# JBLanier/stratego_env

Measured on AMD Instinct MI355X. Metric: env steps/sec, higher is better.
Workload: dtype u8

## Files before the change

stratego_env_amd/csrc/sgx_choose.h:

```cpp
#pragma once

namespace {

constexpr int CHOOSE_BITS = 23;
constexpr uint32_t CHOOSE_ONE = 1u << CHOOSE_BITS;

template <class G, int VEC>
struct ChooseGeo {
    static constexpr int NA = G::NA;
    static constexpr int NCH = (NA + VEC - 1) / VEC;
    static constexpr int ROWS = (NCH + G::LPG - 1) / G::LPG;
    static constexpr bool CACHE = ROWS * VEC <= 72;
    static constexpr int WAVES = 4, GAMES = WAVES * G::GPW;
};

__device__ __forceinline__ uint32_t choose_weight(float l, float mx, float scale) {
    const uint32_t w = (uint32_t)exp2f(fmaf(l - mx, scale, (float)CHOOSE_BITS));
    return l == mx ? CHOOSE_ONE : w;
}

template <class G>
__device__ __forceinline__ uint32_t gsum(uint32_t c) {
    if constexpr (G::LPG == 64) {
        int x = (int)c;
        x += dpp_or_zero<0x111>(x);
        x += dpp_or_zero<0x112>(x);
        x += dpp_or_zero<0x114>(x);
        x += dpp_or_zero<0x118>(x);
        return (uint32_t)__builtin_amdgcn_readlane(x, 15) + (uint32_t)__builtin_amdgcn_readlane(x, 31) +
               (uint32_t)__builtin_amdgcn_readlane(x, 47) + (uint32_t)__builtin_amdgcn_readlane(x, 63);
    } else {
        return (uint32_t)glane<G>(gscan_incl<G>((int)c), G::LPG - 1);
    }
}

template <class G>
__device__ __forceinline__ float gmax(float x) {
#pragma unroll
    for (int o = G::LPG / 2; o > 0; o >>= 1) x = fmaxf(x, __shfl_xor(x, o, G::LPG));
    return x;
}

template <int R_, int C_, int VEC, bool BITS>
__global__ __launch_bounds__(256) void choose_kernel(const KParams P, const float *__restrict__ logits, const void *__restrict__ mask, const float scale,
                                                     int32_t *__restrict__ actions) {
    using G = Geo<R_, C_>;
    using CG = ChooseGeo<G, VEC>;
    constexpr int NA = CG::NA, ROWS = CG::ROWS, LPG = G::LPG;
    __shared__ uint32_t rowtot[CG::GAMES][CG::CACHE ? 1 : ROWS];
    const int lane = threadIdx.x & (LPG - 1), slot = threadIdx.x / LPG;
    const int64_t env = blockIdx.x * (int64_t)CG::GAMES + slot;
    if (env >= P.n_envs) return;
    const float *lg = logits + env * (int64_t)NA;
    const uint8_t *mb = BITS ? nullptr : reinterpret_cast<const uint8_t *>(mask) + env * (int64_t)NA;
    const uint32_t *mw = BITS ? reinterpret_cast<const uint32_t *>(mask) + env * (int64_t)G::MB_WORDS : nullptr;
    const int4 sc = rec_scal<G>(P.boards, P.rec_bytes, env)[0];

    auto load_row = [&](int j, float (&v)[VEC], bool stream) {
        const int ch = j * LPG + lane, i = ch * VEC;
#pragma unroll
        for (int e = 0; e < VEC; ++e) v[e] = -INFINITY;
        if (i >= NA) return;
        uint32_t vm;
        if constexpr (VEC == 4) {
            const f32x4 q = stream ? __builtin_nontemporal_load(reinterpret_cast<const f32x4 *>(lg) + ch) : reinterpret_cast<const f32x4 *>(lg)[ch];
            v[0] = q.x; v[1] = q.y; v[2] = q.z; v[3] = q.w;
            if constexpr (BITS) vm = (mw[i >> 5] >> (i & 31)) & 15u;
            else {
                const uint32_t m4 = reinterpret_cast<const uint32_t *>(mb)[ch];
                vm = ((m4 & 0xFFu) ? 1u : 0u) | ((m4 & 0xFF00u) ? 2u : 0u) | ((m4 & 0xFF0000u) ? 4u : 0u) | ((m4 & 0xFF000000u) ? 8u : 0u);
            }
        } else {
            v[0] = stream ? __builtin_nontemporal_load(lg + i) : lg[i];
            if constexpr (BITS) vm = (mw[i >> 5] >> (i & 31)) & 1u;
            else vm = mb[i] ? 1u : 0u;
        }
#pragma unroll
        for (int e = 0; e < VEC; ++e)
            if (!((vm >> e) & 1u) || !(v[e] == v[e])) v[e] = -INFINITY;
    };
    auto chunk_sum = [&](const float (&v)[VEC], float mx) {
        uint32_t c = 0;
#pragma unroll
        for (int e = 0; e < VEC; ++e) c += choose_weight(v[e], mx, scale);
        return c;
    };

    float cv[CG::CACHE ? ROWS : 1][VEC];
    float mx = -INFINITY;
    if constexpr (CG::CACHE) {
#pragma unroll
        for (int j = 0; j < ROWS; ++j) load_row(j, cv[j], true);
#pragma unroll
        for (int j = 0; j < ROWS; ++j)
#pragma unroll
            for (int e = 0; e < VEC; ++e) mx = fmaxf(mx, cv[j][e]);
    } else {
        for (int j = 0; j < ROWS; ++j) {
            float v[VEC];
            load_row(j, v, false);
#pragma unroll
            for (int e = 0; e < VEC; ++e) mx = fmaxf(mx, v[e]);
        }
    }
    mx = gmax<G>(mx);
    if (mx == -INFINITY) {
        if (lane == 0) actions[env] = -1;
        return;
    }

    const uint64_t r = sgx_rng(P.seed, (uint64_t)(P.env_id_offset + env), (uint64_t)sc.w, STREAM_ACTION, (uint32_t)sc.x);
    unsigned long long total = 0, target = 0, before = 0;
    int jr = 0;
    if constexpr (CG::CACHE) {
        uint32_t t[ROWS];
#pragma unroll
        for (int j = 0; j < ROWS; ++j) { t[j] = gsum<G>(chunk_sum(cv[j], mx)); total += t[j]; }
        target = __umul64hi((r >> 32) << 32, total);
        bool found = false;
#pragma unroll
        for (int j = 0; j < ROWS; ++j) {
            if (!found && before + t[j] > target) { jr = j; found = true; }
            if (!found) before += t[j];
        }
    } else {
        for (int j = 0; j < ROWS; ++j) {
            float v[VEC];
            load_row(j, v, false);
            const uint32_t t = gsum<G>(chunk_sum(v, mx));
            if (lane == 0) rowtot[slot][j] = t;
            total += t;
        }
        wave_sync<G>();
        target = __umul64hi((r >> 32) << 32, total);
        for (int j = 0; j < ROWS; ++j) {
            const uint32_t t = rowtot[slot][j];
            if (before + t > target) { jr = j; break; }
            before += t;
        }
    }
    float v[VEC];
    load_row(jr, v, false);
    uint32_t w[VEC], c = 0;
#pragma unroll
    for (int e = 0; e < VEC; ++e) { w[e] = choose_weight(v[e], mx, scale); c += w[e]; }
    const unsigned long long incl = before + (unsigned long long)(uint32_t)gscan_incl<G>((int)c);
    const unsigned long long hit = gballot<G>(incl > target);
    const int l = __ffsll((long long)hit) - 1;
    if (lane == l) {
        unsigned long long cum = incl - c;
        int pick = VEC - 1;
        bool found = false;
#pragma unroll
        for (int e = 0; e < VEC; ++e) {
            cum += w[e];
            if (!found && cum > target) { pick = e; found = true; }
        }
        actions[env] = (jr * LPG + lane) * VEC + pick;
    }
}

}
```

Baseline: 260.8 million.

## Load masks first and skip logit loads and reductions for fully masked rows

The action sampler now reads the legal-action mask for a group of rows first, then fetches logits only for lanes with legal actions. Rows where no lane in the wave has a legal action skip the max, the weight computation and the group-sum reduction. Uncached rows are processed in fixed-size groups so loads can batch. This targets sparse Stratego masks where most logits are illegal, at the cost of extra ballots, bit packing and more complex control flow.

```diff
diff --git a/stratego_env_amd/csrc/sgx_choose.h b/stratego_env_amd/csrc/sgx_choose.h
--- a/stratego_env_amd/csrc/sgx_choose.h
+++ b/stratego_env_amd/csrc/sgx_choose.h
@@ -12,6 +12,8 @@
     static constexpr int ROWS = (NCH + G::LPG - 1) / G::LPG;
     static constexpr bool CACHE = ROWS * VEC <= 72;
     static constexpr int WAVES = 4, GAMES = WAVES * G::GPW;
+    static constexpr int GR = CACHE ? ROWS : VEC == 4 ? 8 : 16;
+    static constexpr int NG = (ROWS + GR - 1) / GR, VW = (GR * VEC + 31) / 32, RW = (GR + 31) / 32;
 };
 
 __device__ __forceinline__ uint32_t choose_weight(float l, float mx, float scale) {
@@ -56,29 +58,58 @@
     const uint32_t *mw = BITS ? reinterpret_cast<const uint32_t *>(mask) + env * (int64_t)G::MB_WORDS : nullptr;
     const int4 sc = rec_scal<G>(P.boards, P.rec_bytes, env)[0];
 
-    auto load_row = [&](int j, float (&v)[VEC], bool stream) {
+    auto load_valid = [&](int j) -> uint32_t {
         const int ch = j * LPG + lane, i = ch * VEC;
-#pragma unroll
-        for (int e = 0; e < VEC; ++e) v[e] = -INFINITY;
-        if (i >= NA) return;
-        uint32_t vm;
+        if (i >= NA) return 0u;
+        if constexpr (BITS) return (mw[i >> 5] >> (i & 31)) & ((1u << VEC) - 1u);
+        else if constexpr (VEC == 4) {
+            const uint32_t m4 = reinterpret_cast<const uint32_t *>(mb)[ch];
+            return ((m4 & 0xFFu) ? 1u : 0u) | ((m4 & 0xFF00u) ? 2u : 0u) | ((m4 & 0xFF0000u) ? 4u : 0u) | ((m4 & 0xFF000000u) ? 8u : 0u);
+        } else return mb[i] ? 1u : 0u;
+    };
+    float ninf = -INFINITY;
+    asm volatile("" : "+v"(ninf));
+    auto wave_any = [](bool pred) { return __ballot(pred) != 0ull; };
+    auto load_logits = [&](int j, uint32_t ld, bool any, float (&v)[VEC], bool stream) {
+#pragma unroll
+        for (int e = 0; e < VEC; ++e) v[e] = ninf;
+        if (!any || ld == 0u) return;
+        const int ch = j * LPG + lane;
         if constexpr (VEC == 4) {
             const f32x4 q = stream ? __builtin_nontemporal_load(reinterpret_cast<const f32x4 *>(lg) + ch) : reinterpret_cast<const f32x4 *>(lg)[ch];
             v[0] = q.x; v[1] = q.y; v[2] = q.z; v[3] = q.w;
-            if constexpr (BITS) vm = (mw[i >> 5] >> (i & 31)) & 15u;
-            else {
-                const uint32_t m4 = reinterpret_cast<const uint32_t *>(mb)[ch];
-                vm = ((m4 & 0xFFu) ? 1u : 0u) | ((m4 & 0xFF00u) ? 2u : 0u) | ((m4 & 0xFF0000u) ? 4u : 0u) | ((m4 & 0xFF000000u) ? 8u : 0u);
-            }
-        } else {
-            v[0] = stream ? __builtin_nontemporal_load(lg + i) : lg[i];
-            if constexpr (BITS) vm = (mw[i >> 5] >> (i & 31)) & 1u;
-            else vm = mb[i] ? 1u : 0u;
-        }
+        } else v[0] = stream ? __builtin_nontemporal_load(lg + ch) : lg[ch];
+    };
+    auto mask_logits = [&](uint32_t vm, float (&v)[VEC]) {
 #pragma unroll
         for (int e = 0; e < VEC; ++e)
             if (!((vm >> e) & 1u) || !(v[e] == v[e])) v[e] = -INFINITY;
     };
+    auto bits_of = [](const uint32_t *b, int k) { return (b[k * VEC / 32] >> (k * VEC % 32)) & ((1u << VEC) - 1u); };
+    auto row_any = [](const uint32_t *ra, int k) { return ((ra[k / 32] >> (k % 32)) & 1u) != 0u; };
+    auto load_group = [&](int j0, float (&v)[CG::GR][VEC], uint32_t (&vb)[CG::VW], uint32_t (&ra)[CG::RW], bool stream) {
+        uint32_t ld[CG::VW];
+#pragma unroll
+        for (int w = 0; w < CG::VW; ++w) vb[w] = 0u;
+#pragma unroll
+        for (int w = 0; w < CG::RW; ++w) ra[w] = 0u;
+#pragma unroll
+        for (int k = 0; k < CG::GR; ++k) vb[k * VEC / 32] |= load_valid(j0 + k) << (k * VEC % 32);
+#pragma unroll
+        for (int w = 0; w < CG::VW; ++w) {
+            ld[w] = vb[w];
+            asm volatile("" : "+v"(ld[w]));
+        }
+#pragma unroll
+        for (int k = 0; k < CG::GR; ++k) {
+            const bool any = wave_any(bits_of(ld, k) != 0u);
+            ra[k / 32] |= (any ? 1u : 0u) << (k % 32);
+            load_logits(j0 + k, bits_of(ld, k), any, v[k], stream);
+        }
+#pragma unroll
+        for (int k = 0; k < CG::GR; ++k)
+            if (row_any(ra, k)) mask_logits(bits_of(vb, k), v[k]);
+    };
     auto chunk_sum = [&](const float (&v)[VEC], float mx) {
         uint32_t c = 0;
 #pragma unroll
@@ -86,22 +117,17 @@
         return c;
     };
 
-    float cv[CG::CACHE ? ROWS : 1][VEC];
+    float cv[CG::GR][VEC];
+    uint32_t vb[CG::VW], ra[CG::RW];
     float mx = -INFINITY;
-    if constexpr (CG::CACHE) {
-#pragma unroll
-        for (int j = 0; j < ROWS; ++j) load_row(j, cv[j], true);
-#pragma unroll
-        for (int j = 0; j < ROWS; ++j)
-#pragma unroll
-            for (int e = 0; e < VEC; ++e) mx = fmaxf(mx, cv[j][e]);
-    } else {
-        for (int j = 0; j < ROWS; ++j) {
-            float v[VEC];
-            load_row(j, v, false);
-#pragma unroll
-            for (int e = 0; e < VEC; ++e) mx = fmaxf(mx, v[e]);
-        }
+    for (int g = 0; g < CG::NG; ++g) {
+        load_group(g * CG::GR, cv, vb, ra, CG::CACHE);
+#pragma unroll
+        for (int k = 0; k < CG::GR; ++k)
+            if (row_any(ra, k)) {
+#pragma unroll
+                for (int e = 0; e < VEC; ++e) mx = fmaxf(mx, cv[k][e]);
+            }
     }
     mx = gmax<G>(mx);
     if (mx == -INFINITY) {
@@ -115,7 +141,7 @@
     if constexpr (CG::CACHE) {
         uint32_t t[ROWS];
 #pragma unroll
-        for (int j = 0; j < ROWS; ++j) { t[j] = gsum<G>(chunk_sum(cv[j], mx)); total += t[j]; }
+        for (int j = 0; j < ROWS; ++j) { t[j] = row_any(ra, j) ? gsum<G>(chunk_sum(cv[j], mx)) : 0u; total += t[j]; }
         target = __umul64hi((r >> 32) << 32, total);
         bool found = false;
 #pragma unroll
@@ -124,12 +150,17 @@
             if (!found) before += t[j];
         }
     } else {
-        for (int j = 0; j < ROWS; ++j) {
-            float v[VEC];
-            load_row(j, v, false);
-            const uint32_t t = gsum<G>(chunk_sum(v, mx));
-            if (lane == 0) rowtot[slot][j] = t;
-            total += t;
+        for (int g = 0; g < CG::NG; ++g) {
+            load_group(g * CG::GR, cv, vb, ra, false);
+#pragma unroll
+            for (int k = 0; k < CG::GR; ++k) {
+                const int j = g * CG::GR + k;
+                if (j < ROWS) {
+                    const uint32_t t = row_any(ra, k) ? gsum<G>(chunk_sum(cv[k], mx)) : 0u;
+                    if (lane == 0) rowtot[slot][j] = t;
+                    total += t;
+                }
+            }
         }
         wave_sync<G>();
         target = __umul64hi((r >> 32) << 32, total);
@@ -140,7 +171,16 @@
         }
     }
     float v[VEC];
-    load_row(jr, v, false);
+    uint32_t vr;
+    if constexpr (CG::CACHE) {
+        uint32_t word = vb[0];
+#pragma unroll
+        for (int w = 1; w < CG::VW; ++w)
+            if (jr * VEC / 32 == w) word = vb[w];
+        vr = (word >> (jr * VEC % 32)) & ((1u << VEC) - 1u);
+    } else vr = load_valid(jr);
+    load_logits(jr, vr, wave_any(vr != 0u), v, false);
+    mask_logits(vr, v);
     uint32_t w[VEC], c = 0;
 #pragma unroll
     for (int e = 0; e < VEC; ++e) { w[e] = choose_weight(v[e], mx, scale); c += w[e]; }
```

New measurement: 260.7 million (median of 2 runs). About the same (-0.0%).
